# MVME-HBUT/Faster-OreFSDet

Measured on NVIDIA B200. Metric: query_images_per_sec, higher is better.
Workload: dtype f32

## Files before the change

### faster_orefsdet_b200/csrc/conv_tc.cu

```cuda
#include <cuda_fp16.h>

#include "common.cuh"
#include "split_format.cuh"
#include "tc05.cuh"

namespace fod {

using namespace tc;

namespace cvt {

constexpr int kTileH = 8, kTileW = 16;
constexpr int kChunk = 32;
constexpr int kQStages = 3, kStages = 6, kAccStages = 2;
constexpr int kPartChunks = 16;
constexpr uint32_t kQStageStrideS1 = ((kTileH + 2) * (kTileW + 2) * 128 + 1023) / 1024 * 1024;
constexpr uint32_t kBPlaneMax = 64 * 64;
constexpr uint32_t kBStageBytes = 2 * kBPlaneMax;
constexpr uint32_t kSlabBytes = 128 * 128;

constexpr uint32_t kOffQ = 0;
constexpr uint32_t kOffB = kOffQ + kQStages * kQStageStrideS1;
constexpr uint32_t kOffSum = kOffB + kStages * kBStageBytes;
constexpr uint32_t kOffBias = kOffSum + 4 * kSlabBytes;
// ... 35 lines not shown
  float* y_amax;
  float* colsum;
  float* colsumsq;
  const float* res;
  int res_h, res_w, res_shift;
  int tiles_x, tiles_per_img, tiles_total;
  int taps, stride, per_tap;
  int cin_chunks, chunks, parts, chunks_per_part;
  int n_groups, n_group, nhalf, ncol32, cout;
  int relu, num_pairs, pair_units, n_amax, ho, wo;
  int x_amax_stride;
  int y_amax_per_image;
  const float* x_actual;
  float* y_bound;
  float y_l1, y_beta;
};

struct TmemA {
  const float* a_gate;
  const float* a_shift;
  int a_relu, in_h, in_w, cin;
  int ksize, halo_w;
  uint32_t q_stage_bytes, q_stage_stride;
  int x_presplit;
  int x_presplit_from;
  int slice_ch[8];
};

struct SmemA {
  uint32_t a_box_bytes, b_stage_bytes, off_b, off_sum;
  int b_stages;
};

struct Unit {
  int n, tt, ty, tx;
  int ch0;
  bool store;
};
__device__ __forceinline__ bool has_unit(const Params& P, int pair, int i) { return i * P.num_pairs + pair < P.pair_units; }
__device__ __forceinline__ Unit unit_of(const Params& P, int pair, uint32_t rank, int i) {
  const int pu = i * P.num_pairs + pair, t = 2 * (pu / P.n_groups) + (int)rank;
  const int tc = min(t, P.tiles_total - 1);
  Unit u;
  u.store = t < P.tiles_total;
  u.n = tc / P.tiles_per_img;
  u.tt = tc - u.n * P.tiles_per_img;
  u.ty = u.tt / P.tiles_x;
  u.tx = u.tt - u.ty * P.tiles_x;
  u.ch0 = (pu % P.n_groups) * P.n_group;
  return u;
}
__device__ __forceinline__ bool ends_part(int pc, int lc, int chunks_per_part, int chunks) {
  return pc == chunks_per_part - 1 || lc == chunks - 1;
}
__device__ __forceinline__ uint32_t ring_stage(uint32_t g, uint32_t n) { return g % n; }
__device__ __forceinline__ uint32_t ring_phase(uint32_t g, uint32_t n) { return (g / n) & 1u; }
__device__ __forceinline__ uint32_t ring_next(uint32_t s, uint32_t n) { return s + 1 == n ? 0u : s + 1; }
__device__ __forceinline__ void flag_publish(uint32_t flag, uint32_t n) {
  asm volatile("st.release.cta.shared.u32 [%0], %1;" ::"r"(flag), "r"(n) : "memory");
}
__device__ __forceinline__ void flag_wait(uint32_t flag, uint32_t& upto, uint32_t g) {
  while (upto <= g) {
    uint32_t v;
    asm volatile("ld.acquire.cta.shared.u32 %0, [%1];" : "=r"(v) : "r"(flag) : "memory");
    upto = __shfl_sync(0xffffffffu, v, 0);
  }
}
__device__ __forceinline__ float image_bound(const Params& P, int n) {
  float amax = 0.f;
  const float* col = P.x_amax + (P.x_amax_stride ? n : 0);
  const int step = P.x_amax_stride ? P.x_amax_stride : 1;
  for (int i = 0; i < P.n_amax; ++i) amax = fmaxf(amax, __ldg(col + (size_t)i * step));
  return amax;
}
__device__ __forceinline__ uint32_t pair_setup(const Params& P, uint8_t* tmem_ptr, int warp, int lane) {
  if (warp == kWarpAlloc) {
    tmem_alloc<2>(smem_u32(tmem_ptr), kTmemCols);
    tmem_relinquish<2>();
  }
  if (warp == kWarpTma && lane == 0) {
    tma_prefetch_desc(&P.in_map);
// ... 1 lines not shown
    tma_prefetch_desc(&P.whi_map);
    tma_prefetch_desc(&P.wlo_map);
  }
  tc_fence_before();
  cluster_sync();
  tc_fence_after();
  return *reinterpret_cast<volatile uint32_t*>(tmem_ptr);
}
__device__ __forceinline__ void pair_teardown(int warp, uint32_t tmem_base) {
  __syncwarp();
  tc_fence_before();
  cluster_sync();
  if (warp == kWarpAlloc) tmem_dealloc<2>(tmem_base, kTmemCols);
}

template <int kTaps>
__device__ __forceinline__ void weight_producer(const Params& P, int pair, uint32_t rank, uint32_t dst0, uint32_t stage_bytes,
                                                uint32_t stages, uint32_t full0, uint32_t free0) {
#ifdef FOD_DBG
  long long* const dbg_buf = (pair == 0 && rank == 0) ? g_dbg : nullptr;
  constexpr int lane = 0;
#endif
  const uint32_t full_leader = map_to_cta(full0, 0);
  const uint32_t plane = (uint32_t)P.nhalf * 64u;
  uint32_t g = 0;
  for (int i = 0; has_unit(P, pair, i); ++i) {
    const int row0 = unit_of(P, pair, rank, i).ch0 + (int)rank * P.nhalf;
    for (int cc = 0; cc < P.cin_chunks; ++cc)
      for (int tap0 = 0; tap0 < P.taps; tap0 += kTaps, ++g) {
        const uint32_t s = ring_stage(g, stages);
        DBG_STAMP(0, g, 0);
        mbar_wait(free0 + 8u * s, ring_phase(g, stages) ^ 1);
        DBG_STAMP(0, g, 1);
        if (rank == 0) mbar_arrive_expect_tx(full0 + 8u * s, 4 * kTaps * plane);
#pragma unroll
        for (int k = 0; k < kTaps; ++k) {
          const int k0 = ((tap0 + k) * P.cin_chunks + cc) * kChunk;
          const uint32_t dst = dst0 + s * stage_bytes + k * 2 * plane;
          tma_load_2d_2sm(dst, &P.whi_map, full_leader + 8u * s, k0, row0);
          tma_load_2d_2sm(dst + plane, &P.wlo_map, full_leader + 8u * s, k0, row0);
        }
      }
  }
}

template <int kEpiWarps>
__device__ __forceinline__ void epilogue(const Params& P, uint8_t* smem, uint32_t off_sum, uint32_t off_bias, uint32_t acc_full0,
                                         uint32_t acc_empty0, uint32_t tmem_acc, int warp, int lane, int pair, uint32_t rank) {
  const uint32_t sbase = smem_u32(smem);
  const int qd = warp & 3, sp = (warp - kWarpEpi0) >> 2;
  constexpr int sstep = kEpiWarps / 4;
  const int m = qd * 32 + lane;
  const uint32_t acc_empty_leader = map_to_cta(acc_empty0, 0);
  const bool issuer = (warp == kWarpEpi0 && lane == 0);
  const uint32_t row_s = sbase + off_sum + (uint32_t)((m >> 3) * 1024 + (m & 7) * 128);
  const uint32_t bias_s = sbase + off_bias;
  const int ncol32 = P.ncol32, parts = P.parts;
  const float w_inv = __ldg(P.w_inv);
  float vmax = 0.f;
  uint32_t gp = 0;
  for (int i = 0; has_unit(P, pair, i); ++i) {
    const Unit u = unit_of(P, pair, rank, i);
    const float x_bound = image_bound(P, u.n);
    float xs, xs_inv;
    pow2_scale(x_bound, xs, xs_inv);
    const float rescale = xs_inv * w_inv;
// ... 13 lines not shown
    if (issuer) tma_store_wait_read<0>();
    named_bar_sync(1, 32 * kEpiWarps);
    if (sp == 0) reinterpret_cast<float*>(smem + off_bias)[m] = (P.bias && u.ch0 + m < P.cout) ? __ldg(P.bias + u.ch0 + m) : 0.f;
    named_bar_sync(1, 32 * kEpiWarps);
#pragma unroll 1
    for (int part = 0; part < parts; ++part, ++gp) {
      const uint32_t as_ = ring_stage(gp, kAccStages);
      mbar_wait(acc_full0 + 8u * as_, ring_phase(gp, kAccStages));
      tc_fence_after();
      const uint32_t trow = tmem_acc + ((uint32_t)(qd * 32) << 16) + as_ * 128u;
      if (sp >= ncol32) {
        __syncwarp();
        if (lane == 0) mbar_arrive_remote(acc_empty_leader + 8u * as_);
      }
      const bool final = part == parts - 1;
#pragma unroll 1
      for (int j = sp; j < ncol32; j += sstep) {
        uint32_t v[32];
        tmem_ld32(trow + j * 32, v);
        tmem_wait_ld();
        if (j + sstep >= ncol32) {
          tc_fence_before();
          __syncwarp();
          if (lane == 0) mbar_arrive_remote(acc_empty_leader + 8u * as_);
        }
        const uint32_t slab = row_s + (uint32_t)j * kSlabBytes;
        float4 xv[8];
#pragma unroll
        for (int c4 = 0; c4 < 8; ++c4) {
          const int cb = u.ch0 + j * 32 + c4 * 4;
          float4 x = make_float4(__uint_as_float(v[c4 * 4 + 0]), __uint_as_float(v[c4 * 4 + 1]), __uint_as_float(v[c4 * 4 + 2]),
                                 __uint_as_float(v[c4 * 4 + 3]));
          if (part > 0) {
            const float4 r = lds4s(slab + (uint32_t)((c4 ^ (m & 7)) << 4));
            x.x += r.x; x.y += r.y; x.z += r.z; x.w += r.w;
          }
          if (final) {
            const float4 bb = lds4s(bias_s + (j * 32 + c4 * 4) * 4);
            x.x = fmaf(x.x, rescale, bb.x); x.y = fmaf(x.y, rescale, bb.y);
            x.z = fmaf(x.z, rescale, bb.z); x.w = fmaf(x.w, rescale, bb.w);
            if (res_px && cb < P.cout) {
              const float4 rv = ldg4(res_px + cb);
              x.x += rv.x; x.y += rv.y; x.z += rv.z; x.w += rv.w;
            }
            if (P.relu) {
              x.x = fmaxf(x.x, 0.f); x.y = fmaxf(x.y, 0.f); x.z = fmaxf(x.z, 0.f); x.w = fmaxf(x.w, 0.f);
            }
            if (P.y_amax && px_valid) {
              if (cb + 0 < P.cout) vmax = fmaxf(vmax, fabsf(x.x));
              if (cb + 1 < P.cout) vmax = fmaxf(vmax, fabsf(x.y));
              if (cb + 2 < P.cout) vmax = fmaxf(vmax, fabsf(x.z));
              if (cb + 3 < P.cout) vmax = fmaxf(vmax, fabsf(x.w));
            }
          }
          xv[c4] = x;
        }
        if (final && ysplit != 0.f) {
#pragma unroll
          for (int c = 0; c < 4; ++c) {
            uint32_t hi[4], lo[4];
            split_f16x2(xv[2 * c].x * ysplit, xv[2 * c].y * ysplit, hi[0], lo[0]);
            split_f16x2(xv[2 * c].z * ysplit, xv[2 * c].w * ysplit, hi[1], lo[1]);
            split_f16x2(xv[2 * c + 1].x * ysplit, xv[2 * c + 1].y * ysplit, hi[2], lo[2]);
            split_f16x2(xv[2 * c + 1].z * ysplit, xv[2 * c + 1].w * ysplit, hi[3], lo[3]);
            const int hp = (c >> 1) * 4 + (c & 1);
            asm volatile("st.shared.v4.b32 [%0], {%1,%2,%3,%4};" ::"r"(slab + (uint32_t)((hp ^ (m & 7)) << 4)), "r"(hi[0]), "r"(hi[1]),
                         "r"(hi[2]), "r"(hi[3]) : "memory");
            asm volatile("st.shared.v4.b32 [%0], {%1,%2,%3,%4};" ::"r"(slab + (uint32_t)(((hp + 2) ^ (m & 7)) << 4)), "r"(lo[0]),
                         "r"(lo[1]), "r"(lo[2]), "r"(lo[3]) : "memory");
          }
        } else {
#pragma unroll
          for (int c4 = 0; c4 < 8; ++c4) sts4s(slab + (uint32_t)((c4 ^ (m & 7)) << 4), xv[c4]);
        }
      }
    }
    if (P.y_amax && P.y_amax_per_image) {
      const uint32_t wmax = __reduce_max_sync(0xffffffffu, __float_as_uint(vmax));
      if (lane == 0 && wmax) atomicMax(reinterpret_cast<unsigned int*>(P.y_amax + u.n), wmax);
      vmax = 0.f;
    }
    fence_proxy_async_smem();
    named_bar_sync(1, 32 * kEpiWarps);
    if (issuer && u.store) {
      for (int j = 0; j < ncol32 && u.ch0 + j * 32 < P.cout; ++j)
        tma_store_4d(&P.out_map, sbase + off_sum + j * kSlabBytes, u.ch0 + j * 32, u.tx * kTileW, u.ty * kTileH, u.n);
      tma_store_commit();
    }
    if (P.colsum && u.store && sp == 0 && qd < ncol32) {
// ... 74 lines not shown
      const int pad = T.ksize >> 1, loads = P.per_tap ? P.taps : 1;
      for (int i = 0; has_unit(P, pair, i); ++i) {
        const Unit u = unit_of(P, pair, rank, i);
        const int x0 = u.tx * kTileW * P.stride - pad, y0 = u.ty * kTileH * P.stride - pad;
        for (int cc = 0; cc < P.cin_chunks; ++cc)
          for (int tap = 0; tap < loads; ++tap, ++g) {
            const uint32_t s = ring_stage(g, kQStages);
            const int dy = tap / T.ksize, dx = tap - dy * T.ksize;
            mbar_wait(q_empty(s), ring_phase(g, kQStages) ^ 1);
            mbar_arrive_expect_tx(q_full(s), T.q_stage_bytes);
            tma_load_4d(sbase + kOffQ + s * T.q_stage_stride, &P.in_map, q_full(s), cc * kChunk, x0 + dx, y0 + dy, u.n);
          }
      }
    }
  } else if (warp == kWarpTmaB) {
    if (lane == 0) weight_producer<1>(P, pair, rank, sbase + kOffB, kBStageBytes, kStages, ready(0), st_free(0));
  } else if (warp == kWarpMma) {
    if (rank == 0) {
      const uint32_t idesc = idesc_f16(256, P.n_group);
      const uint32_t plane16 = ((uint32_t)P.nhalf * 64u) >> 4;
      const int cpp = P.chunks_per_part, chunks = P.chunks;
      const uint64_t bhi0 = smem_desc_k_sw64(sbase + kOffB);
      const uint32_t a00 = tmem_base + kColA, d0 = tmem_base + kColAcc;
      uint64_t bhi = bhi0;
      uint32_t a0 = a00, d = d0, sf = st_free(0), af = acc_full(0);
      uint32_t upto = 0, g = 0, s = 0;
      int pc = 0, as_ = 0;
      for (int i = 0; has_unit(P, pair, i); ++i) {
        for (int lc = 0; lc < chunks; ++lc, ++g) {
          DBG_STAMP(1, g, 0);
          flag_wait(flag, upto, g);
          tc_fence_after();
          DBG_STAMP(1, g, 1);
          const bool last = ends_part(pc, lc, cpp, chunks);
          if (elect_one()) {
            const uint64_t blo = bhi + plane16;
#pragma unroll
            for (int ks = 0; ks < 2; ++ks) {
              const uint32_t ah = a0 + ks * 8, al = ah + 16;
              const uint64_t boff = (uint64_t)((ks * 32) >> 4);
              mma_f16_ts<2>(d, ah, bhi + boff, idesc, (pc | ks) ? 1u : 0u);
              mma_f16_ts<2>(d, al, bhi + boff, idesc, 1u);
              mma_f16_ts<2>(d, ah, blo + boff, idesc, 1u);
            }
            mma_commit_pair(sf, 3);
            if (last) mma_commit_pair(af, 3);
          }
          __syncwarp();
          DBG_STAMP(1, g, 2);
// ... 10 lines not shown
        }
      }
    }
  } else if (warp == kWarpAlloc) {
    if (rank == 0 && lane == 0) {
      uint32_t g = 0, gp = 0;
      for (int i = 0; has_unit(P, pair, i); ++i) {
        int pc = 0;
        for (int lc = 0; lc < P.chunks; ++lc, ++g) {
          DBG_STAMP(2, g, 0);
          if (pc == 0) mbar_wait(acc_empty(ring_stage(gp, kAccStages)), ring_phase(gp, kAccStages) ^ 1);
          DBG_STAMP(2, g, 1);
          mbar_wait(ready(ring_stage(g, kStages)), ring_phase(g, kStages));
          DBG_STAMP(2, g, 3);
          flag_publish(flag, g + 1);
          const bool last = ends_part(pc, lc, P.chunks_per_part, P.chunks);
          pc = last ? 0 : pc + 1;
          gp += last;
        }
      }
    }
  } else if (warp < kWarpConv0) {
    epilogue<4>(P, smem, kOffSum, kOffBias, acc_full(0), acc_empty(0), tmem_base + kColAcc, warp, lane, pair, rank);
  } else {
    const int cw = warp - kWarpConv0;
    const int qd = cw & 3, half = (cw >> 2) & 1, set = cw >> 3;
    const int m = qd * 32 + lane;
    const int py = m >> 4, px = m & 15;
    const bool per_tap = P.per_tap != 0;
    const bool direct = per_tap || P.taps == 1;
    const uint32_t ready_leader = map_to_cta(ready(0), 0);
// ... 59 lines not shown

    for (int i = 0; has_unit(P, pair, i); ++i) {
      const Unit u = unit_of(P, pair, rank, i);
      pow2_scale(image_bound(P, u.n), xs, xs_inv);
      in_y0 = u.ty * kTileH * P.stride - (ksz >> 1);
      in_x0 = u.tx * kTileW * P.stride - (ksz >> 1);
      for (int cc = 0; cc < P.cin_chunks; ++cc) {
        if (T.a_gate) gate_row = T.a_gate + (size_t)u.n * T.cin + cc * kChunk;
        if (T.a_shift) shift_row = T.a_shift + (size_t)u.n * T.cin + cc * kChunk;
        const int ch16 = cc * kChunk + half * 16;
        const bool pre = direct && ch16 >= T.x_presplit_from;
        __half2 pre_mult = __float2half2_rn(1.f);
        if (pre) {
          int k = P.n_amax - 1;
          while (k > 0 && ch16 < T.slice_ch[k]) --k;
          const int step = P.x_amax_stride ? P.x_amax_stride : 1;
          float sk, sk_inv;
          pow2_scale(__ldg(P.x_amax + (size_t)k * step + (P.x_amax_stride ? u.n : 0)), sk, sk_inv);
          pre_mult = __float2half2_rn(xs * sk_inv);
        }
        uint32_t qs = ring_stage(gq, kQStages);
        uint32_t qt = sbase + kOffQ + qs * T.q_stage_stride;
        if (!per_tap) {
          mbar_wait(q_full(qs), ring_phase(gq, kQStages));
          if (!direct && !T.x_presplit) convert_stage(qt);
        }
        int dy = 0, dx = 0;
        for (int tap = 0; tap < P.taps; ++tap, ++g) {
          if (per_tap) {
            qs = ring_stage(gq, kQStages);
            qt = sbase + kOffQ + qs * T.q_stage_stride;
            mbar_wait(q_full(qs), ring_phase(gq, kQStages));
          }
// ... 59 lines not shown
            ++gq;
          }
        }
        if (!per_tap) {
          __syncwarp();
          if (lane == 0) mbar_arrive(q_empty(qs));
          ++gq;
        }
      }
    }
  }
  pair_teardown(warp, tmem_base);
}

constexpr int kAStagesS = 2;
constexpr int kEpiWarpsS = 8;
constexpr int kThreadsS = (kWarpEpi0 + kEpiWarpsS) * 32;
constexpr uint32_t kRowBytesS1 = 16 * 128;
constexpr uint32_t kMaxDynSmem = 232448;
constexpr uint32_t kNumBarsS = 2 * kAStagesS + 2 * kStages + 2 * kAccStages;
__host__ __device__ constexpr uint32_t smem_a_tail_bytes(int ncol32) { return ncol32 * kSlabBytes + 128 * 4 + kNumBarsS * 8 + 16; }

__global__ void __launch_bounds__(kThreadsS, 1) conv_tc_kernel_smem(const __grid_constant__ Params P, const __grid_constant__ SmemA L) {
  extern __shared__ uint8_t smem_raw[];
  uint8_t* smem = reinterpret_cast<uint8_t*>((reinterpret_cast<uintptr_t>(smem_raw) + 1023) & ~uintptr_t(1023));
  const uint32_t sbase = smem_u32(smem);
  const int tid = threadIdx.x, warp = __shfl_sync(0xffffffffu, tid >> 5, 0), lane = tid & 31;
  const uint32_t rank = blockIdx.x & 1;
  const int pair = blockIdx.x >> 1;
  const uint32_t off_bias = L.off_sum + (uint32_t)P.ncol32 * kSlabBytes, off_bars = off_bias + 128 * 4;
  const uint32_t off_tmem_ptr = off_bars + kNumBarsS * 8;
  const uint32_t bar0 = sbase + off_bars, flag = sbase + off_tmem_ptr + 8;
  auto a_full = [&](int s) { return bar0 + 8u * s; };
  auto a_empty = [&](int s) { return bar0 + 8u * (kAStagesS + s); };
  auto b_full = [&](int s) { return bar0 + 8u * (2 * kAStagesS + s); };
  auto b_free = [&](int s) { return bar0 + 8u * (2 * kAStagesS + kStages + s); };
  auto acc_full = [&](int s) { return bar0 + 8u * (2 * kAStagesS + 2 * kStages + s); };
  auto acc_empty = [&](int s) { return bar0 + 8u * (2 * kAStagesS + 2 * kStages + kAccStages + s); };
  if (tid == 0) {
    for (int s = 0; s < kAStagesS; ++s) {
      mbar_init(a_full(s), 1);
      mbar_init(a_empty(s), 1);
    }
    for (int s = 0; s < L.b_stages; ++s) {
      mbar_init(b_full(s), 1);
      mbar_init(b_free(s), 1);
    }
    for (int s = 0; s < kAccStages; ++s) {
      mbar_init(acc_full(s), 1);
      mbar_init(acc_empty(s), 2 * kEpiWarpsS);
    }
    *reinterpret_cast<volatile uint32_t*>(smem + off_tmem_ptr + 8) = 0;
    fence_barrier_init();
  }
  const uint32_t tmem_base = pair_setup(P, smem + off_tmem_ptr, warp, lane);

  const bool per_row_a = P.per_tap != 0;
  const uint32_t a_stage_bytes = 3 * L.a_box_bytes;
  if (warp == kWarpTma) {
    if (lane == 0) {
      const uint32_t a_full_leader = map_to_cta(a_full(0), 0);
      uint32_t ga = 0;
      for (int i = 0; has_unit(P, pair, i); ++i) {
        const Unit u = unit_of(P, pair, rank, i);
        const int x0 = u.tx * kTileW * P.stride - 1, y0 = u.ty * kTileH * P.stride - 1;
        for (int cc = 0; cc < P.cin_chunks; ++cc)
          for (int dy = 0; dy < 3; dy += per_row_a ? 1 : 3, ++ga) {
            const uint32_t s = ring_stage(ga, kAStagesS);
            mbar_wait(a_empty(s), ring_phase(ga, kAStagesS) ^ 1);
            if (rank == 0) mbar_arrive_expect_tx(a_full(s), 2 * a_stage_bytes);
            for (int dx = 0; dx < 3; ++dx)
              tma_load_4d_2sm(sbase + s * a_stage_bytes + dx * L.a_box_bytes, &P.in_map, a_full_leader + 8u * s,
                              cc * kChunk, x0 + dx, y0 + dy, u.n);
          }
      }
    }
  } else if (warp == kWarpTmaB) {
    if (lane == 0) weight_producer<3>(P, pair, rank, sbase + L.off_b, L.b_stage_bytes, L.b_stages, b_full(0), b_free(0));
  } else if (warp == kWarpMma) {
    if (rank == 0) {
      const uint32_t idesc = idesc_f16(256, P.n_group);
      const uint32_t plane16 = ((uint32_t)P.nhalf * 64u) >> 4, tap16 = 2 * plane16, bstep16 = L.b_stage_bytes >> 4;
      const uint32_t box16 = L.a_box_bytes >> 4, astep16 = a_stage_bytes >> 4, row16 = per_row_a ? 0u : kRowBytesS1 >> 4;
      const int cpp = P.chunks_per_part, chunks = P.chunks;
      const uint64_t a_desc0 = smem_desc_k_sw128(sbase), b_desc0 = smem_desc_k_sw64(sbase + L.off_b);
      const uint32_t d0 = tmem_base + kColAcc;
      uint64_t a_desc = a_desc0, b_desc = b_desc0;
      uint32_t d = d0, af = acc_full(0), sf = b_free(0), qf = a_empty(0);
      uint32_t upto = 0, g = 0, sb = 0, sa = 0;
      int pc = 0, as_ = 0;
      for (int i = 0; has_unit(P, pair, i); ++i) {
        int lc = 0;
        for (int cc = 0; cc < P.cin_chunks; ++cc)
          for (int dy = 0; dy < 3; ++dy, ++g) {
            flag_wait(flag, upto, g);
            tc_fence_after();
            const uint64_t a_row = a_desc + (uint64_t)(dy * row16);
#pragma unroll 1
            for (int dx = 0; dx < 3; ++dx, ++lc) {
              const bool last = ends_part(pc, lc, cpp, chunks);
              if (elect_one()) {
                const uint64_t a = a_row + dx * box16, bhi = b_desc + dx * tap16, blo = bhi + plane16;
#pragma unroll
                for (int ks = 0; ks < 2; ++ks) {
                  const uint64_t ah = a + (uint64_t)(ks * 4), al = ah + 2u, boff = (uint64_t)(ks * 2);
                  mma_f16_ss<2>(d, ah, bhi + boff, idesc, (pc | ks) ? 1u : 0u);
                  mma_f16_ss<2>(d, al, bhi + boff, idesc, 1u);
                  mma_f16_ss<2>(d, ah, blo + boff, idesc, 1u);
                }
                if (last) mma_commit_pair(af, 3);
              }
              __syncwarp();
              pc = last ? 0 : pc + 1;
              if (last) {
                as_ ^= 1;
                d = d0 + (uint32_t)as_ * 128u;
                af = acc_full(as_);
              }
            }
            const bool a_done = per_row_a || dy == 2;
            if (elect_one()) {
              mma_commit_pair(sf, 3);
              if (a_done) mma_commit_pair(qf, 3);
            }
            __syncwarp();
            sb = ring_next(sb, L.b_stages);
            b_desc = b_desc0 + sb * bstep16;
            sf = b_free(sb);
            if (a_done) {
              sa = ring_next(sa, kAStagesS);
              a_desc = a_desc0 + sa * astep16;
              qf = a_empty(sa);
            }
          }
      }
    }
  } else if (warp == kWarpAlloc) {
    if (rank == 0 && lane == 0) {
      uint32_t g = 0, ga = 0, gp = 0;
      for (int i = 0; has_unit(P, pair, i); ++i) {
        int pc = 0, lc = 0;
        for (int cc = 0; cc < P.cin_chunks; ++cc)
          for (int dy = 0; dy < 3; ++dy, ++g) {
            for (int dx = 0; dx < 3; ++dx, ++lc) {
              if (pc == 0) mbar_wait(acc_empty(ring_stage(gp, kAccStages)), ring_phase(gp, kAccStages) ^ 1);
              const bool last = ends_part(pc, lc, P.chunks_per_part, P.chunks);
              pc = last ? 0 : pc + 1;
              gp += last;
            }
            if (per_row_a || dy == 0) {
              mbar_wait(a_full(ring_stage(ga, kAStagesS)), ring_phase(ga, kAStagesS));
              ++ga;
            }
            mbar_wait(b_full(ring_stage(g, L.b_stages)), ring_phase(g, L.b_stages));
            flag_publish(flag, g + 1);
          }
      }
    }
  } else {
    epilogue<kEpiWarpsS>(P, smem, L.off_sum, off_bias, acc_full(0), acc_empty(0), tmem_base + kColAcc, warp, lane, pair, rank);
  }
  pair_teardown(warp, tmem_base);
}

__global__ void absmax_kernel(const float* __restrict__ x, size_t n, float* __restrict__ out) {
  x += (size_t)blockIdx.y * n;
  out += blockIdx.y;
  float m = 0.f;
  const size_t n4 = n >> 2;
  for (size_t i = (size_t)blockIdx.x * blockDim.x + threadIdx.x; i < n4; i += (size_t)gridDim.x * blockDim.x) {
    const float4 v = ldg4(x + i * 4);
// ... 118 lines not shown
  FOD_REQUIRE(w_oihw && packed, "fod_conv2d_pack_weights: null pointer");
  FOD_REQUIRE(cout > 0 && cin > 0 && (ksize == 1 || ksize == 3), "fod_conv2d_pack_weights: bad sizes");
  FOD_REQUIRE((((uintptr_t)w_oihw | (uintptr_t)packed) & 15) == 0, "fod_conv2d_pack_weights: pointers must be 16-byte aligned");
  const int cin_pad = (cin + 31) / 32 * 32;
  const size_t plane = (size_t)cout * ksize * ksize * cin_pad;
  __half* hi = reinterpret_cast<__half*>(packed);
  float* tail = packed + plane;
  int rc = fod_absmax(w_oihw, (size_t)cout * cin * ksize * ksize, tail + 2, stream);
  if (rc != FOD_OK) return rc;
  const unsigned blocks = (unsigned)((plane + 255) / 256 < 4096 ? (plane + 255) / 256 : 4096);
  cvt::pack_weights_kernel<<<blocks, 256, 0, as_stream(stream)>>>(w_oihw, cout, cin, ksize, cin_pad, hi, hi + plane, tail);
  FOD_CUDA_LAUNCH_CHECK("fod_conv2d_pack_weights");
  return FOD_OK;
}

static bool smem_a_layout(const cvt::Params& P, bool presplit_one_scale, cvt::SmemA& L) {
  if (!presplit_one_scale || !(P.n_group <= 96 || (P.stride == 2 && P.n_group == 128))) return false;
  L.a_box_bytes = (uint32_t)(cvt::kTileW * (P.per_tap ? cvt::kTileH : cvt::kTileH + 2) * 128);
  L.b_stage_bytes = (uint32_t)(6 * P.nhalf * 64 + 1023) / 1024 * 1024;
  L.off_b = cvt::kAStagesS * 3 * L.a_box_bytes;
  const long room = (long)cvt::kMaxDynSmem - 1024 - L.off_b - cvt::smem_a_tail_bytes(P.ncol32);
  L.b_stages = (int)(room / (long)L.b_stage_bytes < cvt::kStages ? room / (long)L.b_stage_bytes : cvt::kStages);
  L.off_sum = L.off_b + (uint32_t)L.b_stages * L.b_stage_bytes;
  return L.b_stages >= 2;
}

static int conv2d_nhwc_impl(const float* x, int n, int h, int w, int cin, long x_pixel_stride, const float* x_amax,
                            int n_amax, int amax_per_image, const float* packed, const float* bias, int cout, int ksize, int stride,
                            int relu, float* y, long y_pixel_stride, float* y_amax, const float* residual,
                            int residual_upsample2, const float* a_gate, const float* a_shift, int a_relu, float* colsum,
                            float* colsumsq, const float* x_actual, float* y_bound, float y_l1, float y_beta,
                            int x_presplit_from, const int* slice_ch, fod_stream_t stream) {
  FOD_REQUIRE((((uintptr_t)a_gate | (uintptr_t)a_shift | (uintptr_t)colsum | (uintptr_t)colsumsq) & 15) == 0,
              "fod_conv2d_nhwc: a_gate / a_shift / colsum / colsumsq must be 16-byte aligned");
  FOD_REQUIRE((!a_gate && !a_shift) || cin % 32 == 0, "fod_conv2d_nhwc: a_gate / a_shift need cin to be a multiple of 32");
  FOD_REQUIRE(!colsumsq || colsum, "fod_conv2d_nhwc: colsumsq needs colsum");
  FOD_REQUIRE(x && packed && y && x_amax, "fod_conv2d_nhwc: null pointer");
// ... 64 lines not shown
  tm.in_h = h;
  tm.in_w = w;
  prm.colsum = colsum;
  prm.colsumsq = colsumsq;
  tm.cin = cin;
  prm.res = residual;
  prm.res_shift = residual_upsample2 ? 1 : 0;
  prm.res_h = residual_upsample2 ? (ho + 1) / 2 : ho;
  prm.res_w = residual_upsample2 ? (wo + 1) / 2 : wo;
  prm.tiles_x = (wo + cvt::kTileW - 1) / cvt::kTileW;
  prm.tiles_per_img = prm.tiles_x * ((ho + cvt::kTileH - 1) / cvt::kTileH);
  const long tiles = (long)n * prm.tiles_per_img;
  FOD_REQUIRE(tiles * prm.n_groups < (1L << 30), "fod_conv2d_nhwc: too many tiles");
  prm.tiles_total = (int)tiles;
  prm.pair_units = (int)((tiles + 1) / 2) * prm.n_groups;
  cvt::SmemA sm = {};
  const bool smem_a = smem_a_layout(prm, tm.x_presplit || (stride == 2 && x_presplit_from == 0 && n_amax == 1), sm);
  int rc = make_nhwc_map(&prm.in_map, x, n, h, w, cin, x_pixel_stride, cvt::kChunk, smem_a && !per_tap ? cvt::kTileW : halo_w,
                         halo_h, stride, CU_TENSOR_MAP_SWIZZLE_128B);
  if (rc != FOD_OK) return rc;
  rc = make_nhwc_map(&prm.out_map, y, n, ho, wo, cout, y_pixel_stride, cvt::kChunk, cvt::kTileW, cvt::kTileH, 1,
                     CU_TENSOR_MAP_SWIZZLE_128B);
  if (rc != FOD_OK) return rc;
  const long ktot = (long)prm.taps * cin_pad;
  const __half* whi = reinterpret_cast<const __half*>(packed);
  rc = make_matrix_map_f16(&prm.whi_map, whi, cout, ktot, cvt::kChunk, prm.nhalf);
  if (rc != FOD_OK) return rc;
  rc = make_matrix_map_f16(&prm.wlo_map, whi + (size_t)cout * ktot, cout, ktot, cvt::kChunk, prm.nhalf);
  if (rc != FOD_OK) return rc;
  prm.w_inv = packed + (size_t)cout * ktot;
  int dev = 0, sms = 0;
  FOD_CUDA_CALL(cudaGetDevice(&dev));
// ... 47 lines not shown
```

Before: 6833.

## Route 1x1 multi-slice convs through SMEM-A path with per-slice scaled partial sums

Adds a per-slice mode for 1x1 convolutions whose input is a concatenation of separately scaled channel slices. These convs now use the shared-memory A-operand kernel, with per-chunk channel offsets, half-chunk MMA skipping, and partial-sum boundaries at slice ends. Each partial is rescaled by its own slice bound in the epilogue instead of going through the TMEM conversion path. It also lets the 8-warp epilogue keep running sums in registers instead of a shared-memory slab, and sizes the A ring from available shared memory. In exchange it adds more partial accumulations and epilogue passes, plus more complex barrier and stage bookkeeping.

```diff
diff --git a/faster_orefsdet_b200/csrc/conv_tc.cu b/faster_orefsdet_b200/csrc/conv_tc.cu
--- a/faster_orefsdet_b200/csrc/conv_tc.cu
+++ b/faster_orefsdet_b200/csrc/conv_tc.cu
@@ -73,6 +73,9 @@
   const float* x_actual;
   float* y_bound;
   float y_l1, y_beta;
+  uint64_t slice_ends;
+  int part_scaled;
+  int8_t part_slice[16];
 };
 
 struct TmemA {
@@ -88,7 +91,10 @@
 
 struct SmemA {
   uint32_t a_box_bytes, b_stage_bytes, off_b, off_sum;
-  int b_stages;
+  int a_stages, b_stages;
+  int sub;
+  uint64_t half_chunks;
+  int16_t chunk_ch[64];
 };
 
 struct Unit {
@@ -109,9 +115,10 @@
   u.ch0 = (pu % P.n_groups) * P.n_group;
   return u;
 }
-__device__ __forceinline__ bool ends_part(int pc, int lc, int chunks_per_part, int chunks) {
-  return pc == chunks_per_part - 1 || lc == chunks - 1;
-}
+__host__ __device__ __forceinline__ bool ends_part(const Params& P, int pc, int lc) {
+  return pc == P.chunks_per_part - 1 || lc == P.chunks - 1 || (lc < 64 && ((P.slice_ends >> lc) & 1));
+}
+__device__ __forceinline__ int dense_k0(const Params& P, int lc) { return ((lc % P.taps) * P.cin_chunks + lc / P.taps) * kChunk; }
 __device__ __forceinline__ uint32_t ring_stage(uint32_t g, uint32_t n) { return g % n; }
 __device__ __forceinline__ uint32_t ring_phase(uint32_t g, uint32_t n) { return (g / n) & 1u; }
 __device__ __forceinline__ uint32_t ring_next(uint32_t s, uint32_t n) { return s + 1 == n ? 0u : s + 1; }
@@ -124,6 +131,9 @@
     asm volatile("ld.acquire.cta.shared.u32 %0, [%1];" : "=r"(v) : "r"(flag) : "memory");
     upto = __shfl_sync(0xffffffffu, v, 0);
   }
+}
+__device__ __forceinline__ float row_bound(const Params& P, int n, int k) {
+  return __ldg(P.x_amax + (size_t)k * (P.x_amax_stride ? P.x_amax_stride : 1) + (P.x_amax_stride ? n : 0));
 }
 __device__ __forceinline__ float image_bound(const Params& P, int n) {
   float amax = 0.f;
@@ -155,9 +165,9 @@
   if (warp == kWarpAlloc) tmem_dealloc<2>(tmem_base, kTmemCols);
 }
 
-template <int kTaps>
-__device__ __forceinline__ void weight_producer(const Params& P, int pair, uint32_t rank, uint32_t dst0, uint32_t stage_bytes,
-                                                uint32_t stages, uint32_t full0, uint32_t free0) {
+template <class K0>
+__device__ __forceinline__ void weight_producer(const Params& P, int pair, uint32_t rank, int sub, K0 k0_of, uint32_t dst0,
+                                                uint32_t stage_bytes, uint32_t stages, uint32_t full0, uint32_t free0) {
 #ifdef FOD_DBG
   long long* const dbg_buf = (pair == 0 && rank == 0) ? g_dbg : nullptr;
   constexpr int lane = 0;
@@ -167,21 +177,20 @@
   uint32_t g = 0;
   for (int i = 0; has_unit(P, pair, i); ++i) {
     const int row0 = unit_of(P, pair, rank, i).ch0 + (int)rank * P.nhalf;
-    for (int cc = 0; cc < P.cin_chunks; ++cc)
-      for (int tap0 = 0; tap0 < P.taps; tap0 += kTaps, ++g) {
-        const uint32_t s = ring_stage(g, stages);
-        DBG_STAMP(0, g, 0);
-        mbar_wait(free0 + 8u * s, ring_phase(g, stages) ^ 1);
-        DBG_STAMP(0, g, 1);
-        if (rank == 0) mbar_arrive_expect_tx(full0 + 8u * s, 4 * kTaps * plane);
-#pragma unroll
-        for (int k = 0; k < kTaps; ++k) {
-          const int k0 = ((tap0 + k) * P.cin_chunks + cc) * kChunk;
-          const uint32_t dst = dst0 + s * stage_bytes + k * 2 * plane;
-          tma_load_2d_2sm(dst, &P.whi_map, full_leader + 8u * s, k0, row0);
-          tma_load_2d_2sm(dst + plane, &P.wlo_map, full_leader + 8u * s, k0, row0);
-        }
-      }
+    for (int lc = 0; lc < P.chunks; lc += sub, ++g) {
+      const int nb = min(sub, P.chunks - lc);
+      const uint32_t s = ring_stage(g, stages);
+      DBG_STAMP(0, g, 0);
+      mbar_wait(free0 + 8u * s, ring_phase(g, stages) ^ 1);
+      DBG_STAMP(0, g, 1);
+      if (rank == 0) mbar_arrive_expect_tx(full0 + 8u * s, 4 * nb * plane);
+      for (int k = 0; k < nb; ++k) {
+        const int k0 = k0_of(lc + k);
+        const uint32_t dst = dst0 + s * stage_bytes + k * 2 * plane;
+        tma_load_2d_2sm(dst, &P.whi_map, full_leader + 8u * s, k0, row0);
+        tma_load_2d_2sm(dst + plane, &P.wlo_map, full_leader + 8u * s, k0, row0);
+      }
+    }
   }
 }
 
@@ -191,6 +200,9 @@
   const uint32_t sbase = smem_u32(smem);
   const int qd = warp & 3, sp = (warp - kWarpEpi0) >> 2;
   constexpr int sstep = kEpiWarps / 4;
+  constexpr bool kRegSum = kEpiWarps == 8;
+  constexpr int kCols = kRegSum ? 16 : 32;
+  float4 run[2][8];
   const int m = qd * 32 + lane;
   const uint32_t acc_empty_leader = map_to_cta(acc_empty0, 0);
   const bool issuer = (warp == kWarpEpi0 && lane == 0);
@@ -234,65 +246,89 @@
         if (lane == 0) mbar_arrive_remote(acc_empty_leader + 8u * as_);
       }
       const bool final = part == parts - 1;
+      float pscale = 1.f;
+      if (P.part_scaled) {
+        float sk, sk_inv;
+        pow2_scale(row_bound(P, u.n, P.part_slice[part]), sk, sk_inv);
+        pscale = xs * sk_inv;
+      }
+      auto slab_part = [&](int j, float4* run) {
+        const uint32_t slab = row_s + (uint32_t)j * kSlabBytes;
+#pragma unroll
+        for (int h = 0; h < 32 / kCols; ++h) {
+          uint32_t v[kCols];
+          if constexpr (kCols == 16) tmem_ld16(trow + j * 32 + h * 16, v); else tmem_ld32(trow + j * 32, v);
+          tmem_wait_ld();
+          if (h == 32 / kCols - 1 && j + sstep >= ncol32) {
+            tc_fence_before();
+            __syncwarp();
+            if (lane == 0) mbar_arrive_remote(acc_empty_leader + 8u * as_);
+          }
+          float4 xv[kCols / 4];
+#pragma unroll
+          for (int q = 0; q < kCols / 4; ++q) {
+            const int c4 = h * (kCols / 4) + q;
+            const int cb = u.ch0 + j * 32 + c4 * 4;
+            float4 x = make_float4(__uint_as_float(v[q * 4 + 0]), __uint_as_float(v[q * 4 + 1]), __uint_as_float(v[q * 4 + 2]),
+                                   __uint_as_float(v[q * 4 + 3]));
+            if (P.part_scaled) {
+              x.x *= pscale; x.y *= pscale; x.z *= pscale; x.w *= pscale;
+            }
+            if (part > 0) {
+              const float4 r = run ? run[c4] : lds4s(slab + (uint32_t)((c4 ^ (m & 7)) << 4));
+              x.x += r.x; x.y += r.y; x.z += r.z; x.w += r.w;
+            }
+            if (final) {
+              const float4 bb = lds4s(bias_s + (j * 32 + c4 * 4) * 4);
+              x.x = fmaf(x.x, rescale, bb.x); x.y = fmaf(x.y, rescale, bb.y);
+              x.z = fmaf(x.z, rescale, bb.z); x.w = fmaf(x.w, rescale, bb.w);
+              if (res_px && cb < P.cout) {
+                const float4 rv = ldg4(res_px + cb);
+                x.x += rv.x; x.y += rv.y; x.z += rv.z; x.w += rv.w;
+              }
+              if (P.relu) {
+                x.x = fmaxf(x.x, 0.f); x.y = fmaxf(x.y, 0.f); x.z = fmaxf(x.z, 0.f); x.w = fmaxf(x.w, 0.f);
+              }
+              if (P.y_amax && px_valid) {
+                if (cb + 0 < P.cout) vmax = fmaxf(vmax, fabsf(x.x));
+                if (cb + 1 < P.cout) vmax = fmaxf(vmax, fabsf(x.y));
+                if (cb + 2 < P.cout) vmax = fmaxf(vmax, fabsf(x.z));
+                if (cb + 3 < P.cout) vmax = fmaxf(vmax, fabsf(x.w));
+              }
+            }
+            xv[q] = x;
+          }
+          if (run && !final) {
+#pragma unroll
+            for (int q = 0; q < kCols / 4; ++q) run[h * (kCols / 4) + q] = xv[q];
+          } else if (final && ysplit != 0.f) {
+#pragma unroll
+            for (int cq = 0; cq < kCols / 8; ++cq) {
+              const int c = h * (kCols / 8) + cq;
+              uint32_t hi[4], lo[4];
+              split_f16x2(xv[2 * cq].x * ysplit, xv[2 * cq].y * ysplit, hi[0], lo[0]);
+              split_f16x2(xv[2 * cq].z * ysplit, xv[2 * cq].w * ysplit, hi[1], lo[1]);
+              split_f16x2(xv[2 * cq + 1].x * ysplit, xv[2 * cq + 1].y * ysplit, hi[2], lo[2]);
+              split_f16x2(xv[2 * cq + 1].z * ysplit, xv[2 * cq + 1].w * ysplit, hi[3], lo[3]);
+              const int hp = (c >> 1) * 4 + (c & 1);
+              asm volatile("st.shared.v4.b32 [%0], {%1,%2,%3,%4};" ::"r"(slab + (uint32_t)((hp ^ (m & 7)) << 4)), "r"(hi[0]), "r"(hi[1]),
+                           "r"(hi[2]), "r"(hi[3]) : "memory");
+              asm volatile("st.shared.v4.b32 [%0], {%1,%2,%3,%4};" ::"r"(slab + (uint32_t)(((hp + 2) ^ (m & 7)) << 4)), "r"(lo[0]),
+                           "r"(lo[1]), "r"(lo[2]), "r"(lo[3]) : "memory");
+            }
+          } else {
+#pragma unroll
+            for (int q = 0; q < kCols / 4; ++q) sts4s(slab + (uint32_t)(((h * (kCols / 4) + q) ^ (m & 7)) << 4), xv[q]);
+          }
+        }
+      };
+      if constexpr (kRegSum) {
+#pragma unroll
+        for (int k = 0; k < 2; ++k)
+          if (sp + k * sstep < ncol32) slab_part(sp + k * sstep, run[k]);
+      } else {
 #pragma unroll 1
-      for (int j = sp; j < ncol32; j += sstep) {
-        uint32_t v[32];
-        tmem_ld32(trow + j * 32, v);
-        tmem_wait_ld();
-        if (j + sstep >= ncol32) {
-          tc_fence_before();
-          __syncwarp();
-          if (lane == 0) mbar_arrive_remote(acc_empty_leader + 8u * as_);
-        }
-        const uint32_t slab = row_s + (uint32_t)j * kSlabBytes;
-        float4 xv[8];
-#pragma unroll
-        for (int c4 = 0; c4 < 8; ++c4) {
-          const int cb = u.ch0 + j * 32 + c4 * 4;
-          float4 x = make_float4(__uint_as_float(v[c4 * 4 + 0]), __uint_as_float(v[c4 * 4 + 1]), __uint_as_float(v[c4 * 4 + 2]),
-                                 __uint_as_float(v[c4 * 4 + 3]));
-          if (part > 0) {
-            const float4 r = lds4s(slab + (uint32_t)((c4 ^ (m & 7)) << 4));
-            x.x += r.x; x.y += r.y; x.z += r.z; x.w += r.w;
-          }
-          if (final) {
-            const float4 bb = lds4s(bias_s + (j * 32 + c4 * 4) * 4);
-            x.x = fmaf(x.x, rescale, bb.x); x.y = fmaf(x.y, rescale, bb.y);
-            x.z = fmaf(x.z, rescale, bb.z); x.w = fmaf(x.w, rescale, bb.w);
-            if (res_px && cb < P.cout) {
-              const float4 rv = ldg4(res_px + cb);
-              x.x += rv.x; x.y += rv.y; x.z += rv.z; x.w += rv.w;
-            }
-            if (P.relu) {
-              x.x = fmaxf(x.x, 0.f); x.y = fmaxf(x.y, 0.f); x.z = fmaxf(x.z, 0.f); x.w = fmaxf(x.w, 0.f);
-            }
-            if (P.y_amax && px_valid) {
-              if (cb + 0 < P.cout) vmax = fmaxf(vmax, fabsf(x.x));
-              if (cb + 1 < P.cout) vmax = fmaxf(vmax, fabsf(x.y));
-              if (cb + 2 < P.cout) vmax = fmaxf(vmax, fabsf(x.z));
-              if (cb + 3 < P.cout) vmax = fmaxf(vmax, fabsf(x.w));
-            }
-          }
-          xv[c4] = x;
-        }
-        if (final && ysplit != 0.f) {
-#pragma unroll
-          for (int c = 0; c < 4; ++c) {
-            uint32_t hi[4], lo[4];
-            split_f16x2(xv[2 * c].x * ysplit, xv[2 * c].y * ysplit, hi[0], lo[0]);
-            split_f16x2(xv[2 * c].z * ysplit, xv[2 * c].w * ysplit, hi[1], lo[1]);
-            split_f16x2(xv[2 * c + 1].x * ysplit, xv[2 * c + 1].y * ysplit, hi[2], lo[2]);
-            split_f16x2(xv[2 * c + 1].z * ysplit, xv[2 * c + 1].w * ysplit, hi[3], lo[3]);
-            const int hp = (c >> 1) * 4 + (c & 1);
-            asm volatile("st.shared.v4.b32 [%0], {%1,%2,%3,%4};" ::"r"(slab + (uint32_t)((hp ^ (m & 7)) << 4)), "r"(hi[0]), "r"(hi[1]),
-                         "r"(hi[2]), "r"(hi[3]) : "memory");
-            asm volatile("st.shared.v4.b32 [%0], {%1,%2,%3,%4};" ::"r"(slab + (uint32_t)(((hp + 2) ^ (m & 7)) << 4)), "r"(lo[0]),
-                         "r"(lo[1]), "r"(lo[2]), "r"(lo[3]) : "memory");
-          }
-        } else {
-#pragma unroll
-          for (int c4 = 0; c4 < 8; ++c4) sts4s(slab + (uint32_t)((c4 ^ (m & 7)) << 4), xv[c4]);
-        }
+        for (int j = sp; j < ncol32; j += sstep) slab_part(j, nullptr);
       }
     }
     if (P.y_amax && P.y_amax_per_image) {
@@ -397,12 +433,14 @@
       }
     }
   } else if (warp == kWarpTmaB) {
-    if (lane == 0) weight_producer<1>(P, pair, rank, sbase + kOffB, kBStageBytes, kStages, ready(0), st_free(0));
+    if (lane == 0)
+      weight_producer(P, pair, rank, 1, [&](int lc) { return dense_k0(P, lc); }, sbase + kOffB, kBStageBytes, kStages, ready(0),
+                      st_free(0));
   } else if (warp == kWarpMma) {
     if (rank == 0) {
       const uint32_t idesc = idesc_f16(256, P.n_group);
       const uint32_t plane16 = ((uint32_t)P.nhalf * 64u) >> 4;
-      const int cpp = P.chunks_per_part, chunks = P.chunks;
+      const int chunks = P.chunks;
       const uint64_t bhi0 = smem_desc_k_sw64(sbase + kOffB);
       const uint32_t a00 = tmem_base + kColA, d0 = tmem_base + kColAcc;
       uint64_t bhi = bhi0;
@@ -415,7 +453,7 @@
           flag_wait(flag, upto, g);
           tc_fence_after();
           DBG_STAMP(1, g, 1);
-          const bool last = ends_part(pc, lc, cpp, chunks);
+          const bool last = ends_part(P, pc, lc);
           if (elect_one()) {
             const uint64_t blo = bhi + plane16;
 #pragma unroll
@@ -456,7 +494,7 @@
           mbar_wait(ready(ring_stage(g, kStages)), ring_phase(g, kStages));
           DBG_STAMP(2, g, 3);
           flag_publish(flag, g + 1);
-          const bool last = ends_part(pc, lc, P.chunks_per_part, P.chunks);
+          const bool last = ends_part(P, pc, lc);
           pc = last ? 0 : pc + 1;
           gp += last;
         }
@@ -546,9 +584,8 @@
         if (pre) {
           int k = P.n_amax - 1;
           while (k > 0 && ch16 < T.slice_ch[k]) --k;
-          const int step = P.x_amax_stride ? P.x_amax_stride : 1;
           float sk, sk_inv;
-          pow2_scale(__ldg(P.x_amax + (size_t)k * step + (P.x_amax_stride ? u.n : 0)), sk, sk_inv);
+          pow2_scale(row_bound(P, u.n, k), sk, sk_inv);
           pre_mult = __float2half2_rn(xs * sk_inv);
         }
         uint32_t qs = ring_stage(gq, kQStages);
@@ -638,11 +675,12 @@
 }
 
 constexpr int kAStagesS = 2;
+constexpr int kMaxAStagesS = 8;
 constexpr int kEpiWarpsS = 8;
 constexpr int kThreadsS = (kWarpEpi0 + kEpiWarpsS) * 32;
 constexpr uint32_t kRowBytesS1 = 16 * 128;
 constexpr uint32_t kMaxDynSmem = 232448;
-constexpr uint32_t kNumBarsS = 2 * kAStagesS + 2 * kStages + 2 * kAccStages;
+constexpr uint32_t kNumBarsS = 2 * kMaxAStagesS + 2 * kStages + 2 * kAccStages;
 __host__ __device__ constexpr uint32_t smem_a_tail_bytes(int ncol32) { return ncol32 * kSlabBytes + 128 * 4 + kNumBarsS * 8 + 16; }
 
 __global__ void __launch_bounds__(kThreadsS, 1) conv_tc_kernel_smem(const __grid_constant__ Params P, const __grid_constant__ SmemA L) {
@@ -656,13 +694,13 @@
   const uint32_t off_tmem_ptr = off_bars + kNumBarsS * 8;
   const uint32_t bar0 = sbase + off_bars, flag = sbase + off_tmem_ptr + 8;
   auto a_full = [&](int s) { return bar0 + 8u * s; };
-  auto a_empty = [&](int s) { return bar0 + 8u * (kAStagesS + s); };
-  auto b_full = [&](int s) { return bar0 + 8u * (2 * kAStagesS + s); };
-  auto b_free = [&](int s) { return bar0 + 8u * (2 * kAStagesS + kStages + s); };
-  auto acc_full = [&](int s) { return bar0 + 8u * (2 * kAStagesS + 2 * kStages + s); };
-  auto acc_empty = [&](int s) { return bar0 + 8u * (2 * kAStagesS + 2 * kStages + kAccStages + s); };
+  auto a_empty = [&](int s) { return bar0 + 8u * (kMaxAStagesS + s); };
+  auto b_full = [&](int s) { return bar0 + 8u * (2 * kMaxAStagesS + s); };
+  auto b_free = [&](int s) { return bar0 + 8u * (2 * kMaxAStagesS + kStages + s); };
+  auto acc_full = [&](int s) { return bar0 + 8u * (2 * kMaxAStagesS + 2 * kStages + s); };
+  auto acc_empty = [&](int s) { return bar0 + 8u * (2 * kMaxAStagesS + 2 * kStages + kAccStages + s); };
   if (tid == 0) {
-    for (int s = 0; s < kAStagesS; ++s) {
+    for (int s = 0; s < L.a_stages; ++s) {
       mbar_init(a_full(s), 1);
       mbar_init(a_empty(s), 1);
     }
@@ -679,34 +717,42 @@
   }
   const uint32_t tmem_base = pair_setup(P, smem + off_tmem_ptr, warp, lane);
 
-  const bool per_row_a = P.per_tap != 0;
-  const uint32_t a_stage_bytes = 3 * L.a_box_bytes;
+  const bool one_tap = P.taps == 1;
+  const bool per_row_a = P.per_tap != 0 || one_tap;
+  const uint32_t a_stage_bytes = (uint32_t)L.sub * L.a_box_bytes;
+  auto row_dy = [&](int r) { return one_tap ? 0 : r % 3; };
   if (warp == kWarpTma) {
     if (lane == 0) {
       const uint32_t a_full_leader = map_to_cta(a_full(0), 0);
+      const int pad = one_tap ? 0 : 1;
       uint32_t ga = 0;
       for (int i = 0; has_unit(P, pair, i); ++i) {
         const Unit u = unit_of(P, pair, rank, i);
-        const int x0 = u.tx * kTileW * P.stride - 1, y0 = u.ty * kTileH * P.stride - 1;
-        for (int cc = 0; cc < P.cin_chunks; ++cc)
-          for (int dy = 0; dy < 3; dy += per_row_a ? 1 : 3, ++ga) {
-            const uint32_t s = ring_stage(ga, kAStagesS);
-            mbar_wait(a_empty(s), ring_phase(ga, kAStagesS) ^ 1);
-            if (rank == 0) mbar_arrive_expect_tx(a_full(s), 2 * a_stage_bytes);
-            for (int dx = 0; dx < 3; ++dx)
-              tma_load_4d_2sm(sbase + s * a_stage_bytes + dx * L.a_box_bytes, &P.in_map, a_full_leader + 8u * s,
-                              cc * kChunk, x0 + dx, y0 + dy, u.n);
-          }
+        const int x0 = u.tx * kTileW * P.stride - pad, y0 = u.ty * kTileH * P.stride - pad;
+        for (int lc = 0, r = 0; lc < P.chunks; lc += L.sub, ++r) {
+          const int dy = row_dy(r);
+          if (!per_row_a && dy != 0) continue;
+          const int nb = min(L.sub, P.chunks - lc);
+          const uint32_t s = ring_stage(ga, L.a_stages);
+          mbar_wait(a_empty(s), ring_phase(ga, L.a_stages) ^ 1);
+          if (rank == 0) mbar_arrive_expect_tx(a_full(s), 2 * nb * L.a_box_bytes);
+          for (int j = 0; j < nb; ++j)
+            tma_load_4d_2sm(sbase + s * a_stage_bytes + j * L.a_box_bytes, &P.in_map, a_full_leader + 8u * s,
+                            one_tap ? (int)L.chunk_ch[lc + j] : lc / P.taps * kChunk, x0 + (one_tap ? 0 : j), y0 + dy, u.n);
+          ++ga;
+        }
       }
     }
   } else if (warp == kWarpTmaB) {
-    if (lane == 0) weight_producer<3>(P, pair, rank, sbase + L.off_b, L.b_stage_bytes, L.b_stages, b_full(0), b_free(0));
+    if (lane == 0)
+      weight_producer(P, pair, rank, L.sub, [&](int lc) { return one_tap ? (int)L.chunk_ch[lc] : dense_k0(P, lc); },
+                      sbase + L.off_b, L.b_stage_bytes, L.b_stages, b_full(0), b_free(0));
   } else if (warp == kWarpMma) {
     if (rank == 0) {
       const uint32_t idesc = idesc_f16(256, P.n_group);
       const uint32_t plane16 = ((uint32_t)P.nhalf * 64u) >> 4, tap16 = 2 * plane16, bstep16 = L.b_stage_bytes >> 4;
       const uint32_t box16 = L.a_box_bytes >> 4, astep16 = a_stage_bytes >> 4, row16 = per_row_a ? 0u : kRowBytesS1 >> 4;
-      const int cpp = P.chunks_per_part, chunks = P.chunks;
+      const int chunks = P.chunks;
       const uint64_t a_desc0 = smem_desc_k_sw128(sbase), b_desc0 = smem_desc_k_sw64(sbase + L.off_b);
       const uint32_t d0 = tmem_base + kColAcc;
       uint64_t a_desc = a_desc0, b_desc = b_desc0;
@@ -714,71 +760,71 @@
       uint32_t upto = 0, g = 0, sb = 0, sa = 0;
       int pc = 0, as_ = 0;
       for (int i = 0; has_unit(P, pair, i); ++i) {
-        int lc = 0;
-        for (int cc = 0; cc < P.cin_chunks; ++cc)
-          for (int dy = 0; dy < 3; ++dy, ++g) {
-            flag_wait(flag, upto, g);
-            tc_fence_after();
-            const uint64_t a_row = a_desc + (uint64_t)(dy * row16);
+        for (int lc = 0, r = 0; lc < chunks; ++r, ++g) {
+          flag_wait(flag, upto, g);
+          tc_fence_after();
+          const int dy = row_dy(r), nb = min(L.sub, chunks - lc);
+          const uint64_t a_row = a_desc + (uint64_t)(dy * row16);
 #pragma unroll 1
-            for (int dx = 0; dx < 3; ++dx, ++lc) {
-              const bool last = ends_part(pc, lc, cpp, chunks);
-              if (elect_one()) {
-                const uint64_t a = a_row + dx * box16, bhi = b_desc + dx * tap16, blo = bhi + plane16;
-#pragma unroll
-                for (int ks = 0; ks < 2; ++ks) {
-                  const uint64_t ah = a + (uint64_t)(ks * 4), al = ah + 2u, boff = (uint64_t)(ks * 2);
-                  mma_f16_ss<2>(d, ah, bhi + boff, idesc, (pc | ks) ? 1u : 0u);
-                  mma_f16_ss<2>(d, al, bhi + boff, idesc, 1u);
-                  mma_f16_ss<2>(d, ah, blo + boff, idesc, 1u);
-                }
-                if (last) mma_commit_pair(af, 3);
+          for (int j = 0; j < nb; ++j, ++lc) {
+            const bool last = ends_part(P, pc, lc);
+            const bool half = lc < 64 && ((L.half_chunks >> lc) & 1);
+            if (elect_one()) {
+              const uint64_t a = a_row + j * box16, bhi = b_desc + j * tap16, blo = bhi + plane16;
+#pragma unroll
+              for (int ks = 0; ks < 2; ++ks) {
+                if (ks == 1 && half) break;
+                const uint64_t ah = a + (uint64_t)(ks * 4), al = ah + 2u, boff = (uint64_t)(ks * 2);
+                mma_f16_ss<2>(d, ah, bhi + boff, idesc, (pc | ks) ? 1u : 0u);
+                mma_f16_ss<2>(d, al, bhi + boff, idesc, 1u);
+                mma_f16_ss<2>(d, ah, blo + boff, idesc, 1u);
               }
-              __syncwarp();
-              pc = last ? 0 : pc + 1;
-              if (last) {
-                as_ ^= 1;
-                d = d0 + (uint32_t)as_ * 128u;
-                af = acc_full(as_);
-              }
-            }
-            const bool a_done = per_row_a || dy == 2;
-            if (elect_one()) {
-              mma_commit_pair(sf, 3);
-              if (a_done) mma_commit_pair(qf, 3);
+              if (last) mma_commit_pair(af, 3);
             }
             __syncwarp();
-            sb = ring_next(sb, L.b_stages);
-            b_desc = b_desc0 + sb * bstep16;
-            sf = b_free(sb);
-            if (a_done) {
-              sa = ring_next(sa, kAStagesS);
-              a_desc = a_desc0 + sa * astep16;
-              qf = a_empty(sa);
+            pc = last ? 0 : pc + 1;
+            if (last) {
+              as_ ^= 1;
+              d = d0 + (uint32_t)as_ * 128u;
+              af = acc_full(as_);
             }
           }
+          const bool a_done = per_row_a || dy == 2;
+          if (elect_one()) {
+            mma_commit_pair(sf, 3);
+            if (a_done) mma_commit_pair(qf, 3);
+          }
+          __syncwarp();
+          sb = ring_next(sb, L.b_stages);
+          b_desc = b_desc0 + sb * bstep16;
+          sf = b_free(sb);
+          if (a_done) {
+            sa = ring_next(sa, L.a_stages);
+            a_desc = a_desc0 + sa * astep16;
+            qf = a_empty(sa);
+          }
+        }
       }
     }
   } else if (warp == kWarpAlloc) {
     if (rank == 0 && lane == 0) {
       uint32_t g = 0, ga = 0, gp = 0;
       for (int i = 0; has_unit(P, pair, i); ++i) {
-        int pc = 0, lc = 0;
-        for (int cc = 0; cc < P.cin_chunks; ++cc)
-          for (int dy = 0; dy < 3; ++dy, ++g) {
-            for (int dx = 0; dx < 3; ++dx, ++lc) {
-              if (pc == 0) mbar_wait(acc_empty(ring_stage(gp, kAccStages)), ring_phase(gp, kAccStages) ^ 1);
-              const bool last = ends_part(pc, lc, P.chunks_per_part, P.chunks);
-              pc = last ? 0 : pc + 1;
-              gp += last;
-            }
-            if (per_row_a || dy == 0) {
-              mbar_wait(a_full(ring_stage(ga, kAStagesS)), ring_phase(ga, kAStagesS));
-              ++ga;
-            }
-            mbar_wait(b_full(ring_stage(g, L.b_stages)), ring_phase(g, L.b_stages));
-            flag_publish(flag, g + 1);
-          }
+        int pc = 0;
+        for (int lc = 0, r = 0; lc < P.chunks; ++r, ++g) {
+          for (int j = min(L.sub, P.chunks - lc); j > 0; --j, ++lc) {
+            if (pc == 0) mbar_wait(acc_empty(ring_stage(gp, kAccStages)), ring_phase(gp, kAccStages) ^ 1);
+            const bool last = ends_part(P, pc, lc);
+            pc = last ? 0 : pc + 1;
+            gp += last;
+          }
+          if (per_row_a || row_dy(r) == 0) {
+            mbar_wait(a_full(ring_stage(ga, L.a_stages)), ring_phase(ga, L.a_stages));
+            ++ga;
+          }
+          mbar_wait(b_full(ring_stage(g, L.b_stages)), ring_phase(g, L.b_stages));
+          flag_publish(flag, g + 1);
+        }
       }
     }
   } else {
@@ -927,13 +973,26 @@
   return FOD_OK;
 }
 
-static bool smem_a_layout(const cvt::Params& P, bool presplit_one_scale, cvt::SmemA& L) {
+static bool smem_a_layout(const cvt::Params& P, bool presplit_one_scale, bool per_slice, cvt::SmemA& L) {
+  const long room = (long)cvt::kMaxDynSmem - 1024 - cvt::smem_a_tail_bytes(P.ncol32);
+  if (per_slice) {
+    L.sub = 2;
+    L.a_box_bytes = (uint32_t)(cvt::kTileW * cvt::kTileH * 128);
+    L.b_stage_bytes = (uint32_t)(2 * L.sub * P.nhalf * 64 + 1023) / 1024 * 1024;
+    L.b_stages = 2;
+    const long a_fit = (room - (long)L.b_stages * L.b_stage_bytes) / (long)(L.sub * L.a_box_bytes);
+    L.a_stages = (int)(a_fit < cvt::kMaxAStagesS ? a_fit : cvt::kMaxAStagesS);
+    L.off_b = (uint32_t)(L.a_stages * L.sub) * L.a_box_bytes;
+    L.off_sum = L.off_b + (uint32_t)L.b_stages * L.b_stage_bytes;
+    return L.a_stages >= 2;
+  }
   if (!presplit_one_scale || !(P.n_group <= 96 || (P.stride == 2 && P.n_group == 128))) return false;
+  L.sub = 3;
+  L.a_stages = cvt::kAStagesS;
   L.a_box_bytes = (uint32_t)(cvt::kTileW * (P.per_tap ? cvt::kTileH : cvt::kTileH + 2) * 128);
   L.b_stage_bytes = (uint32_t)(6 * P.nhalf * 64 + 1023) / 1024 * 1024;
   L.off_b = cvt::kAStagesS * 3 * L.a_box_bytes;
-  const long room = (long)cvt::kMaxDynSmem - 1024 - L.off_b - cvt::smem_a_tail_bytes(P.ncol32);
-  L.b_stages = (int)(room / (long)L.b_stage_bytes < cvt::kStages ? room / (long)L.b_stage_bytes : cvt::kStages);
+  L.b_stages = (int)((room - L.off_b) / (long)L.b_stage_bytes < cvt::kStages ? (room - L.off_b) / (long)L.b_stage_bytes : cvt::kStages);
   L.off_sum = L.off_b + (uint32_t)L.b_stages * L.b_stage_bytes;
   return L.b_stages >= 2;
 }
@@ -1028,8 +1087,37 @@
   FOD_REQUIRE(tiles * prm.n_groups < (1L << 30), "fod_conv2d_nhwc: too many tiles");
   prm.tiles_total = (int)tiles;
   prm.pair_units = (int)((tiles + 1) / 2) * prm.n_groups;
+  bool per_slice = ksize == 1 && x_presplit_from == 0 && slice_ch && slice_ch[0] == 0;
+  int slice_chunks = 0;
+  for (int k = 0; per_slice && k < n_amax; ++k) {
+    const int end = k + 1 < n_amax ? slice_ch[k + 1] : cin;
+    per_slice = slice_ch[k] % 16 == 0 && end > slice_ch[k];
+    slice_chunks += (end - slice_ch[k] + cvt::kChunk - 1) / cvt::kChunk;
+  }
+  per_slice = per_slice && slice_chunks <= 64;
   cvt::SmemA sm = {};
-  const bool smem_a = smem_a_layout(prm, tm.x_presplit || (stride == 2 && x_presplit_from == 0 && n_amax == 1), sm);
+  const bool smem_a = smem_a_layout(prm, tm.x_presplit || (stride == 2 && x_presplit_from == 0 && n_amax == 1), per_slice, sm);
+  if (smem_a && per_slice) {
+    int lc = 0, slice_of[64];
+    for (int k = 0; k < n_amax; ++k) {
+      const int end = k + 1 < n_amax ? slice_ch[k + 1] : cin;
+      for (int c = slice_ch[k]; c < end; c += cvt::kChunk, ++lc) {
+        sm.chunk_ch[lc] = (int16_t)c;
+        slice_of[lc] = k;
+        if (end - c < cvt::kChunk) sm.half_chunks |= 1ull << lc;
+      }
+      prm.slice_ends |= 1ull << (lc - 1);
+    }
+    prm.chunks = lc;
+    prm.chunks_per_part = cvt::kPartChunks;
+    prm.parts = 0;
+    for (int c = 0, pc = 0; c < lc; ++c) {
+      const bool last = cvt::ends_part(prm, pc, c);
+      if (last) prm.part_slice[prm.parts++] = (int8_t)slice_of[c];
+      pc = last ? 0 : pc + 1;
+    }
+    prm.part_scaled = 1;
+  }
   int rc = make_nhwc_map(&prm.in_map, x, n, h, w, cin, x_pixel_stride, cvt::kChunk, smem_a && !per_tap ? cvt::kTileW : halo_w,
                          halo_h, stride, CU_TENSOR_MAP_SWIZZLE_128B);
   if (rc != FOD_OK) return rc;
```

New measurement: 6020, median of 6. 0.881x the previous value.
